# yeyupiaoling/VoiceprintRecognition-PaddlePaddle

Hardware: AMD Instinct MI355X
Metric: utterances/sec (3 s, 16 kHz) ECAPA-TDNN fwd+AAM (higher is better)
Workload: dtype bf16; 1 GPU; BASELINE configs[1]: ECAPA-TDNN (C=512, MFA 1536, ASP, embd 192) + Kaldi Fbank 80, 3 s @ 16 kHz (T=298), 2796-class cosine head + AAMLoss, eval-mode forward, batch 256 per GPU, inputs resident in HBM, random-init weights; batch_per_gpu=256, global_batch=256, parallelism=dp1 (no collective), streams_per_gpu=2, hip_graph=True, graph_prereplays=40

## Files before the change

### include/vpmi.h

```cpp
#ifndef VPMI_H
#define VPMI_H
#include <stddef.h>
#include <stdint.h>

#ifdef __cplusplus
extern "C" {
#endif

#define VPMI_VERSION 100

typedef struct vp_ctx vp_ctx;
typedef void* vp_stream;

enum { VP_OK = 0, VP_EINVAL = -1, VP_ENOMEM = -2, VP_EHIP = -3, VP_EUNSUP = -4, VP_EWORKSPACE = -5 };
enum { VP_F32 = 0, VP_BF16 = 1,
       VP_F32X3 = 2,
       VP_HL32 = 3 };
enum { VP_PAD_NONE = 0, VP_PAD_REFLECT = 1, VP_PAD_ZERO = 2 };
enum { VP_ACT_NONE = 0, VP_ACT_RELU = 1, VP_ACT_SIGMOID = 2, VP_ACT_TANH = 3,
       VP_ACT_HARDTANH20 = 4,
       VP_ACT_SILU = 5 };

int vp_version(void);
vp_ctx* vp_create(int device);
// ... 99 lines not shown
int vp_se_scale_residual(vp_ctx* ctx, int dtype, const void* x, int ldx, int xoff, const float* s,
                         const void* res, int ldr, int roff, void* out, int ldo, int ooff,
                         int B, int T, int C, vp_stream stream);
int vp_se_scale_residual_shadow(vp_ctx* ctx, const float* x, int ldx, int xoff, const float* s, const float* res, int ldr, int roff,
                                float* out, int ldo, int ooff, void* shadow, int ld_shadow, int shadow_off, int B, int T, int C,
                                vp_stream stream);

int vp_asp_softmax_stats(vp_ctx* ctx, int dtype, const float* logits, const void* x, int ldx, int xoff,
                         int B, int T, int C, float eps, float* pooled, vp_stream stream);

#define VP_MAX_SE_BLOCKS 8
#define VP_MAX_RES2 15

typedef struct {
    const void* w;
    const float* bias;
    const float* bn_scale;
    const float* bn_shift;
    int cin, cout, kw, dil;
    const void* w_hl;
} vp_tdnn_layer;

typedef struct {
    vp_tdnn_layer tdnn1;
    vp_tdnn_layer res2[VP_MAX_RES2];
    vp_tdnn_layer tdnn2;
    const float* se_w1;
    const float* se_b1;
    const float* se_w2;
    const float* se_b2;
} vp_se_res2_block;

typedef struct {
    vp_tdnn_layer tdnn;
    const float* w_ctx;
    const void* conv_w;
    const float* conv_b;
    int C, att;
} vp_asp_weights;

typedef struct {
    int dtype;
    int feat_dim, embd_dim, n_blocks, res2_scale, se_ch;
    vp_tdnn_layer block0;
    vp_se_res2_block blk[VP_MAX_SE_BLOCKS];
    vp_tdnn_layer mfa;
    vp_asp_weights asp;
    const float* fc_w;
    const float* fc_b;
} vp_ecapa_weights;

int vp_res2_chain_fwd(vp_ctx* ctx, const vp_tdnn_layer* layers, int nconv, const void* t1, void* r2, int B, int T, int C,
                      int width, vp_stream stream);
int vp_asp_fused_fwd(vp_ctx* ctx, const void* h, const void* w, const float* bias, const void* x, int ldx, const float* center,
                     int ldc, int B, int T, int C, int att, float eps, float* pooled, vp_stream stream);
int vp_se_gate_fwd(vp_ctx* ctx, const float* psum, const float* shift, int B, int T, int C, int H, const float* w1, const float* b1,
                   const float* w2, const float* b2, float* out, vp_stream stream);
int vp_asp_utt_fwd(vp_ctx* ctx, const void* x, int ldx, const vp_tdnn_layer* tdnn, const float* rowbias, const void* conv_w,
                   const float* conv_b, int B, int T, int C, int att, float eps, float* pooled, vp_stream stream);

int vp_res2_chain_x3_fwd(vp_ctx* ctx, const vp_tdnn_layer* layers, int nconv, const void* t1, void* r2, int B, int T, int C,
                         int width, vp_stream stream);
int vp_res2_chain_x3_plan(int T, int nconv, int dil, int* nsplit, int* tseg, int* tp, int* lds_bytes);
int vp_ecapa_x3_fast_path(const vp_ecapa_weights* w, int B, int T);
int vp_asp_fused_x3_fwd(vp_ctx* ctx, const void* h, const float* w, const float* bias, const void* x, int ldx, const float* center,
                        int ldc, int B, int T, int C, int att, float eps, float* pooled, vp_stream stream);

size_t vp_ecapa_workspace_bytes(const vp_ecapa_weights* w, int B, int T);
int vp_ecapa_fwd(vp_ctx* ctx, const vp_ecapa_weights* w, const void* feats, int B, int T, float* emb,
                 void* ws, size_t ws_bytes, vp_stream stream);

typedef struct {
    int dtype;
    int feat_dim, embd_dim, channels;
    vp_tdnn_layer td[5];
    vp_asp_weights asp;
    const float* lin_w;
    const float* lin_b;
} vp_tdnn_weights;

size_t vp_tdnn_workspace_bytes(const vp_tdnn_weights* w, int B, int T);
int vp_tdnn_fwd(vp_ctx* ctx, const vp_tdnn_weights* w, const void* feats, int B, int T, float* emb,
                void* ws, size_t ws_bytes, vp_stream stream);

#define VP_MAX_CAM_LAYERS 64
#define VP_MAX_CAM_BLOCKS 4

typedef struct {
    vp_tdnn_layer conv1, conv2, shortcut;
    int stride, has_shortcut;
} vp_resblock;

typedef struct {
    const float* bn1_scale;
    const float* bn1_shift;
    vp_tdnn_layer linear1;
    vp_tdnn_layer local;
    const float* ctx_w1;
    const float* ctx_b1;
    const float* ctx_w2;
    const float* ctx_b2;
} vp_cam_layer;

typedef struct {
    const float* bn_scale;
    const float* bn_shift;
// ... 422 lines not shown
```

### voiceprintrecognition-paddlepaddle_amd/csrc/common.h

```cpp
#pragma once
#include <hip/hip_runtime.h>
#include <stdint.h>
#include <stdio.h>
#include <string.h>

#include "../../include/vpmi.h"

struct vp_ctx {
    int device;
    char err[512];
    vp_fbank_opts fb_opts;
    int fb_valid;
    int fb_win, fb_shift, fb_nfft, fb_nmel, fb_nnz;
    float* fb_window;
    float2* fb_twiddle;
    int* fb_mel_start;
    int* fb_mel_bin0;
    float* fb_mel_w;
    float* fb_wpad;
    int fb_f16, fb_rounds, fb_wpad_len, fb_round_off[8], fb_round_max[8];
    vp_mel_opts ms_opts;
    int ms_valid, ms_nnz;
    float* ms_window;
    float2* ms_twiddle;
// ... 63 lines not shown
    o[0] = (bf16_t)v[0]; o[1] = (bf16_t)v[1]; o[2] = (bf16_t)v[2]; o[3] = (bf16_t)v[3];
    *reinterpret_cast<bf16x4*>(p) = o;
}

__device__ __forceinline__ float vp_wave_sum(float v) {
#pragma unroll
    for (int o = 32; o > 0; o >>= 1) v += __shfl_xor(v, o);
    return v;
}
__device__ __forceinline__ float vp_wave_max(float v) {
#pragma unroll
    for (int o = 32; o > 0; o >>= 1) v = fmaxf(v, __shfl_xor(v, o));
    return v;
}

__device__ __forceinline__ unsigned vp_order_key(float s) {
    const unsigned u = __float_as_uint(s);
    return u ^ ((u >> 31) ? 0xffffffffu : 0x80000000u);
}

static inline size_t vp_dtype_size(int dt) { return dt == VP_BF16 ? 2 : 4; }
static inline int vp_storage_dtype(int dt) { return dt == VP_F32X3 ? VP_F32 : dt; }
static inline bool vp_backbone_dtype_ok(int dt) { return dt == VP_F32 || dt == VP_BF16 || dt == VP_F32X3; }

#define VP_CONV_BM 128

int vp_dense_f32_ex(vp_ctx* ctx, const float* a, int lda, const float* w, int w_is_kn, const float* bias,
                    const float* rowscale, const float* colscale, int M, int N, int K, int act, float* out,
                    int ldo, hipStream_t st);
int vp_asp_softmax_stats_ex(vp_ctx* ctx, int dtype, const float* logits, const void* x, int ldx, int xoff,
                            const float* center, int ldc, int B, int T, int C, float eps, float* pooled, hipStream_t st);
struct VpAspBufs { void* h; float* e; float* psum; float* psumsq; float* stats; float* rowbias; float* pooled; };
int vp_run_asp(vp_ctx* ctx, const vp_asp_weights& A, int dtype, const void* x, int ldx, const float* shift,
               int B, int T, const VpAspBufs& w, hipStream_t st);
int vp_asp_utt_bf16(vp_ctx* ctx, const void* x, int ldx, const vp_tdnn_layer* tdnn, const float* rowbias, const void* conv_w,
                    const float* conv_b, int B, int T, int C, int att, float eps, float* pooled, hipStream_t st);
void vp_launch_sum_partials(const float* part, int S, long long n, float* out, hipStream_t st, int Cin = 1, int KW = 1, int batch = 1,
                            int KF = 1);
int vp_conv3x3_c1(vp_ctx* ctx, int dtype, const void* feats, void* out, const float* w, const float* bias,
                  const float* scale, const float* shift, int B, int T, int F, int C, hipStream_t st);
int vp_se_scale_residual_ex(vp_ctx* ctx, int dtype, const void* x, int ldx, int xoff, const float* s,
                            const void* res, int ldr, int roff, void* out, int ldo, int ooff, int B, int T, int C,
                            int relu, hipStream_t st);
int vp_im2col_hl32(vp_ctx* ctx, const float* x, int B, int T, int F, int KW, int dil, int pad, void* out, int Kp, hipStream_t st);
int vp_time_moments(vp_ctx* ctx, int dtype, const void* x, int ldx, int B, int T, int C, float eps, int unbiased,
                    float* stats, hipStream_t st);
int vp_se_gate(vp_ctx* ctx, const float* psum, const float* shift, int B, int T, int C, int H, const float* w1, const float* b1,
               const float* w2, const float* b2, float* out, hipStream_t st);
int vp_copy_cols(vp_ctx* ctx, int dtype, const void* x, int ldx, int xoff, void* y, int ldy, int yoff, long long rows, int C,
                 hipStream_t st);
int vp_aff_combine(vp_ctx* ctx, int dtype, const void* t, int ldt, const void* x, int ldx, int xoff, const void* y, int ldy,
                   int yoff, void* o, int ldo, int ooff, long long rows, int C, hipStream_t st);
int vp_res2_chain_bf16(vp_ctx* ctx, const vp_tdnn_layer* layers, int nconv, const void* t1, void* r2, int B, int T,
                       int C, int width, hipStream_t st);
int vp_res2_chain_x3(vp_ctx* ctx, const vp_tdnn_layer* layers, int nconv, const void* t1, void* r2, int B, int T, int C, int width,
                     hipStream_t st);
bool vp_res2_chain_x3_ok(const vp_tdnn_layer* layers, int nconv, int B, int T, int C, int width);
int vp_asp_fused_x3(vp_ctx* ctx, const void* h, const float* w, const float* bias, const void* x, int ldx, const float* center, int ldc,
                    int B, int T, int C, int att, float eps, float* pooled, hipStream_t st);
int vp_asp_fused_bf16(vp_ctx* ctx, const void* h, const void* w, const float* bias, const void* x, int ldx,
                      const float* center, int ldc, int B, int T, int C, int att, float eps, float* pooled,
                      hipStream_t st);
int vp_row_inv_norm(vp_ctx* ctx, const float* x, int rows, int D, int ld, float eps, float* inv, hipStream_t st);
int vp_reduce_rows(vp_ctx* ctx, const float* v, int n, int mean, float* out, hipStream_t st);
int vp_conv3x3_c32_bf16(vp_ctx* ctx, const void* x, void* y, const vp_tdnn_layer* conv, const void* res, int relu,
                        const vp_tdnn_layer* shortcut, void* y2, int B, int T, int F_in, int stride_f, const void* c1_feats,
                        const float* c1_w, const float* c1_b, const float* c1_scale, const float* c1_shift, hipStream_t st);
int vp_resblock_c32_bf16(vp_ctx* ctx, const void* x, void* y, const vp_tdnn_layer* conv1, const vp_tdnn_layer* conv2, int B, int T, int F,
                         hipStream_t st);
int vp_pointwise_bf16(vp_ctx* ctx, const vp_conv1d_desc* d, int only_where_it_wins, hipStream_t st);
int vp_cam_block_bf16(vp_ctx* ctx, const vp_cam_layer* layers, int n_layers, void* cat, int ld, int ch0, int B, int Tn, int seg_len,
                      int bn_channels, int growth, hipStream_t st);

int vp_fbank_release_tables(vp_ctx* ctx);
int vp_mel_release_tables(vp_ctx* ctx);
int vp_reverb_release_tables(vp_ctx* ctx);

template <typename TO>
__device__ __forceinline__ float vp_tanh_for(float x) {
    if constexpr (sizeof(TO) == 2) {
        const float e = __builtin_amdgcn_exp2f(x * 2.8853900817779268f);
        return 1.f - 2.f * __builtin_amdgcn_rcpf(e + 1.f);
    } else {
        return tanhf(x);
    }
}

template <typename TO>
__device__ __forceinline__ float vp_silu_for(float x) {
    if constexpr (sizeof(TO) == 2) return x * __builtin_amdgcn_rcpf(1.f + __builtin_amdgcn_exp2f(x * -1.4426950408889634f));
    else return x / (1.f + __expf(-x));
}
```

### voiceprintrecognition-paddlepaddle_amd/csrc/ecapa.hip

```cpp
#include "launch.h"

#include <stdlib.h>

namespace {

void tdnn_desc(vp_conv1d_desc& d, const vp_tdnn_layer& L, int dtype, int B, int T_in, int T_out, int pad_mode) {
    vp_layer_desc(d, L, dtype, pad_mode);
    vp_geom_rows(d, B, T_in, T_out);
    d.dilation = L.dil; d.pad_left = pad_mode == VP_PAD_NONE ? 0 : L.dil * (L.kw - 1) / 2;
    d.act = VP_ACT_RELU; d.ldx = d.ldy = 0;
}

}

int vp_run_asp(vp_ctx* ctx, const vp_asp_weights& A, int dtc, const void* x, int ldx, const float* shift,
               int B, int T, const VpAspBufs& w, hipStream_t st) {
    const int C = A.C;
    const int dtype = vp_storage_dtype(dtc);
    int rc = VP_OK;
    if (w.psum) rc = vp_moments_finalize(ctx, w.psum, w.psumsq, shift, B, T, C, 1e-12f, 1, w.stats, st);
    if (rc) return rc;
    if (A.w_ctx) {
        rc = vp_dense_f32_ex(ctx, w.stats, 2 * C, A.w_ctx, 0, nullptr, nullptr, nullptr, B, A.att, 2 * C, VP_ACT_NONE,
                             w.rowbias, A.att, st);
// ... 112 lines not shown
    auto hl_layer = [&](const vp_tdnn_layer& L) {
        tdnn_desc(d, L, VP_F32X3, B, T, T, VP_PAD_REFLECT);
        d.dtype_in = d.dtype_out = VP_HL32; d.w = L.w_hl; d.mfma_bf16 = 2;
    };
    const int Kp0 = (int)vp_align_up((size_t)w->block0.kw * w->block0.cin, 32);
    if (w->block0.w_hl && p.im && w->feat_dim == w->block0.cin && w->block0.cin % 8 == 0) {
        const int pad = w->block0.dil * (w->block0.kw - 1) / 2;
        if ((rc = vp_im2col_hl32(ctx, (const float*)feats, B, T, w->block0.cin, w->block0.kw, w->block0.dil, pad, p.im, Kp0, st))) return rc;
        tdnn_desc(d, w->block0, VP_F32X3, B, T, T, VP_PAD_REFLECT);
        d.dtype_in = d.dtype_out = VP_HL32; d.w = w->block0.w_hl; d.mfma_bf16 = 2;
        d.Cin = Kp0; d.KW = 1; d.dilation = 1; d.pad_left = 0;
        d.x = p.im; d.ldx = Kp0; d.y = p.cat0; d.ldy = C;
    } else {
        tdnn_desc(d, w->block0, VP_F32X3, B, T, T, VP_PAD_REFLECT);
        d.dtype_out = VP_HL32; d.w = w->block0.w; d.mfma_bf16 = 2;
        d.x = feats; d.ldx = w->feat_dim; d.y = p.cat0; d.ldy = C;
    }
    if ((rc = vp_conv1d_fwd(ctx, &d, st))) return rc;
    const void* xin = p.cat0;
    int ld_in = C, off_in = 0;
    for (int i = 0; i < nb; ++i) {
        const vp_se_res2_block& blk = w->blk[i];
        hl_layer(blk.tdnn1);
        d.x = xin; d.ldx = ld_in; d.xoff = off_in; d.y = p.t1; d.ldy = C;
        d.y2 = p.r2; d.ldy2 = C; d.y2off = 0; d.ysplit = width;
        if ((rc = vp_conv1d_fwd(ctx, &d, st))) return rc;
        rc = vp_res2_chain_x3(ctx, blk.res2, sc - 1, p.t1, p.r2, B, T, C, width, st);
        if (rc == VP_EUNSUP) VP_FAIL(ctx, VP_EUNSUP, "ecapa: Res2 chain left the split-precision kernel's range after the shape check");
        if (rc) return rc;
        hl_layer(blk.tdnn2);
        d.x = p.r2; d.ldx = C; d.xoff = 0; d.y = p.t2; d.ldy = C; d.psum = p.psum;
        if ((rc = vp_conv1d_fwd(ctx, &d, st))) return rc;
        if ((rc = vp_se_gate(ctx, p.psum, blk.tdnn2.bn_shift, B, T, C, w->se_ch, blk.se_w1, blk.se_b1, blk.se_w2, blk.se_b2, p.se_s, st)))
            return rc;
        if ((rc = vp_se_scale_residual_ex(ctx, VP_HL32, p.t2, C, 0, p.se_s, xin, ld_in, off_in, p.cat, ldcat, i * C, B, T, C, 0, st))) return rc;
        xin = p.cat; ld_in = ldcat; off_in = i * C;
    }
    hl_layer(w->mfa);
    d.x = p.cat; d.ldx = ldcat; d.y = p.mfa; d.ldy = Cm; d.psum = p.psum; d.psumsq = p.psumsq;
    if ((rc = vp_conv1d_fwd(ctx, &d, st))) return rc;
    VpAspBufs ab{p.h, p.e, p.psum, p.psumsq, p.stats, p.rowbias, p.pooled};
    if ((rc = vp_run_asp(ctx, w->asp, VP_HL32, p.mfa, Cm, w->mfa.bn_shift, B, T, ab, st))) return rc;
    return vp_dense_f32_ex(ctx, p.pooled, 2 * Cm, w->fc_w, 0, w->fc_b, nullptr, nullptr, B, w->embd_dim, 2 * Cm,
                           VP_ACT_NONE, emb, w->embd_dim, st);
}

}

extern "C" {

int vp_res2_chain_fwd(vp_ctx* ctx, const vp_tdnn_layer* layers, int nconv, const void* t1, void* r2, int B, int T, int C,
                      int width, vp_stream stream) {
    if (!ctx || !layers || !t1 || !r2 || B <= 0 || T <= 0 || C <= 0) VP_FAIL(ctx, VP_EINVAL, "res2_chain: bad arguments");
    const int rc = vp_res2_chain_bf16(ctx, layers, nconv, t1, r2, B, T, C, width, (hipStream_t)stream);
    if (rc == VP_EUNSUP) VP_FAIL(ctx, VP_EUNSUP, "res2_chain: shape not covered by the fused kernel (width 64, equal dilations, 2 <= T <= 384)");
    return rc;
}

int vp_asp_utt_fwd(vp_ctx* ctx, const void* x, int ldx, const vp_tdnn_layer* tdnn, const float* rowbias, const void* conv_w,
                   const float* conv_b, int B, int T, int C, int att, float eps, float* pooled, vp_stream stream) {
    if (!ctx || !x || !tdnn || !conv_w || !pooled || B <= 0) VP_FAIL(ctx, VP_EINVAL, "asp_utt: bad arguments");
    const int rc = vp_asp_utt_bf16(ctx, x, ldx, tdnn, rowbias, conv_w, conv_b, B, T, C, att, eps, pooled, (hipStream_t)stream);
    if (rc == VP_EUNSUP) VP_FAIL(ctx, VP_EUNSUP, "asp_utt: shape not covered (attention width 128, C %% 64 == 0, T <= 304, 1x1 TDNN with BatchNorm)");
    return rc;
}

int vp_asp_fused_fwd(vp_ctx* ctx, const void* h, const void* w, const float* bias, const void* x, int ldx, const float* center,
                     int ldc, int B, int T, int C, int att, float eps, float* pooled, vp_stream stream) {
    if (!ctx || !h || !w || !x || !center || !pooled || B <= 0) VP_FAIL(ctx, VP_EINVAL, "asp_fused: bad arguments");
    const int rc = vp_asp_fused_bf16(ctx, h, w, bias, x, ldx, center, ldc, B, T, C, att, eps, pooled, (hipStream_t)stream);
    if (rc == VP_EUNSUP) VP_FAIL(ctx, VP_EUNSUP, "asp_fused: shape not covered (attention width 128, C and ldx multiples of 8, 16-byte aligned)");
    return rc;
}

int vp_res2_chain_x3_fwd(vp_ctx* ctx, const vp_tdnn_layer* layers, int nconv, const void* t1, void* r2, int B, int T, int C,
                         int width, vp_stream stream) {
    if (!ctx || !layers || !t1 || !r2 || B <= 0 || T <= 0 || C <= 0) VP_FAIL(ctx, VP_EINVAL, "res2_chain_x3: bad arguments");
    const int rc = vp_res2_chain_x3(ctx, layers, nconv, t1, r2, B, T, C, width, (hipStream_t)stream);
    if (rc == VP_EUNSUP) VP_FAIL(ctx, VP_EUNSUP, "res2_chain_x3: shape not covered (width 64, equal dilations, split weights present, segments fit the LDS)");
    return rc;
}

int vp_asp_fused_x3_fwd(vp_ctx* ctx, const void* h, const float* w, const float* bias, const void* x, int ldx, const float* center,
                        int ldc, int B, int T, int C, int att, float eps, float* pooled, vp_stream stream) {
    if (!ctx || !h || !w || !bias || !x || !pooled || B <= 0) VP_FAIL(ctx, VP_EINVAL, "asp_fused_x3: bad arguments");
    const int rc = vp_asp_fused_x3(ctx, h, w, bias, x, ldx, center, ldc, B, T, C, att, eps, pooled, (hipStream_t)stream);
    if (rc == VP_EUNSUP) VP_FAIL(ctx, VP_EUNSUP, "asp_fused_x3: shape not covered (attention width 128, C and ldx multiples of 32, 16-byte aligned)");
    return rc;
}

int vp_se_gate_fwd(vp_ctx* ctx, const float* psum, const float* shift, int B, int T, int C, int H, const float* w1, const float* b1,
                   const float* w2, const float* b2, float* out, vp_stream stream) {
    return vp_se_gate(ctx, psum, shift, B, T, C, H, w1, b1, w2, b2, out, (hipStream_t)stream);
}

int vp_ecapa_x3_fast_path(const vp_ecapa_weights* w, int B, int T) {
    if (!w || B <= 0 || T <= 0 || w->dtype != VP_F32X3 || w->n_blocks < 1 || w->n_blocks > VP_MAX_SE_BLOCKS || w->res2_scale < 2 ||
        w->res2_scale - 1 > VP_MAX_RES2)
        return 0;
    return ecapa_hl_ok(w, B, T) ? 1 : 0;
}

size_t vp_ecapa_workspace_bytes(const vp_ecapa_weights* w, int B, int T) {
    if (!w || B <= 0 || T <= 0) return 0;
    EcapaPlan p;
    plan_ecapa(w, B, T, nullptr, p);
    return p.total;
}

int vp_ecapa_fwd(vp_ctx* ctx, const vp_ecapa_weights* w, const void* feats, int B, int T, float* emb,
                 void* ws, size_t ws_bytes, vp_stream stream) {
    if (!ctx || !w || !feats || !emb || B <= 0 || T <= 0) VP_FAIL(ctx, VP_EINVAL, "ecapa: bad arguments");
    int rc = check_ecapa(ctx, w);
    if (rc) return rc;
    EcapaPlan p;
    plan_ecapa(w, B, T, ws, p);
    if (!ws || ws_bytes < p.total) VP_FAIL(ctx, VP_EWORKSPACE, "ecapa: workspace %zu < %zu", ws_bytes, p.total);
    hipStream_t st = (hipStream_t)stream;
    const int dtc = w->dtype, dt = vp_storage_dtype(dtc);
    const int C = w->block0.cout, Cm = w->mfa.cout, nb = w->n_blocks, sc = w->res2_scale;
    const int width = C / sc, ldcat = nb * C;
    vp_conv1d_desc d;
    if (dtc == VP_F32X3 && ecapa_hl_ok(w, B, T)) return ecapa_fwd_hl(ctx, w, feats, B, T, emb, p, st);

    tdnn_desc(d, w->block0, dtc, B, T, T, VP_PAD_REFLECT);
    d.x = feats; d.ldx = w->feat_dim; d.y = p.cat0; d.ldy = C;
    if ((rc = vp_conv1d_fwd(ctx, &d, st))) return rc;

    const void* xin = p.cat0;
    int ld_in = C, off_in = 0;
    for (int i = 0; i < nb; ++i) {
        const vp_se_res2_block& blk = w->blk[i];
        tdnn_desc(d, blk.tdnn1, dtc, B, T, T, VP_PAD_REFLECT);
        d.x = xin; d.ldx = ld_in; d.xoff = off_in; d.y = p.t1; d.ldy = C;
        d.y2 = p.r2; d.ldy2 = C; d.y2off = 0; d.ysplit = width;
        if ((rc = vp_conv1d_fwd(ctx, &d, st))) return rc;
        int fused = VP_EUNSUP;
        static const bool res2_unfused = getenv("VPMI_RES2_UNFUSED") != nullptr;
        if (dt == VP_BF16 && !res2_unfused) fused = vp_res2_chain_bf16(ctx, blk.res2, sc - 1, p.t1, p.r2, B, T, C, width, st);
        if (fused != VP_OK && fused != VP_EUNSUP) return fused;
        void* tin = nullptr;
        void* tout = p.tmpA;
        for (int j = 1; j < sc && fused != VP_OK; ++j) {
            tdnn_desc(d, blk.res2[j - 1], dtc, B, T, T, VP_PAD_REFLECT);
            if (j == 1) { d.x = p.t1; d.ldx = C; d.xoff = width; }
            else { d.x = tin; d.ldx = width; d.xoff = 0; }
            d.y = p.r2; d.ldy = C; d.yoff = j * width;
            if (j + 1 < sc) {
                d.add_in = p.t1; d.ld_add = C; d.add_off = (j + 1) * width;
                d.aux = tout; d.ld_aux = width; d.aux_off = 0;
            }
            if ((rc = vp_conv1d_fwd(ctx, &d, st))) return rc;
            tin = tout;
            tout = (tout == p.tmpA) ? p.tmpB : p.tmpA;
        }
        tdnn_desc(d, blk.tdnn2, dtc, B, T, T, VP_PAD_REFLECT);
        d.x = p.r2; d.ldx = C; d.xoff = 0;
        d.y = p.t2; d.ldy = C; d.psum = p.psum;
        if ((rc = vp_conv1d_fwd(ctx, &d, st))) return rc;
        if ((rc = vp_se_gate(ctx, p.psum, blk.tdnn2.bn_shift, B, T, C, w->se_ch, blk.se_w1, blk.se_b1, blk.se_w2, blk.se_b2,
                             p.se_s, st))) return rc;
        if ((rc = vp_se_scale_residual(ctx, dt, p.t2, C, 0, p.se_s, xin, ld_in, off_in, p.cat, ldcat, i * C, B, T, C, st)))
            return rc;
        xin = p.cat; ld_in = ldcat; off_in = i * C;
    }
    tdnn_desc(d, w->mfa, dtc, B, T, T, VP_PAD_REFLECT);
    d.x = p.cat; d.ldx = ldcat; d.y = p.mfa; d.ldy = Cm; d.psum = p.psum; d.psumsq = p.psumsq;
    if ((rc = vp_conv1d_fwd(ctx, &d, st))) return rc;
    VpAspBufs ab{p.h, p.e, p.psum, p.psumsq, p.stats, p.rowbias, p.pooled};
    if ((rc = vp_run_asp(ctx, w->asp, dtc, p.mfa, Cm, w->mfa.bn_shift, B, T, ab, st))) return rc;
    return vp_dense_f32_ex(ctx, p.pooled, 2 * Cm, w->fc_w, 0, w->fc_b, nullptr, nullptr, B, w->embd_dim, 2 * Cm,
                           VP_ACT_NONE, emb, w->embd_dim, st);
}

static void tdnn_T(const vp_tdnn_weights* w, int T, int Ts[6]) {
    Ts[0] = T;
    for (int i = 0; i < 5; ++i) Ts[i + 1] = Ts[i] - w->td[i].dil * (w->td[i].kw - 1);
}

struct TdnnPlan { void* a; void* b; void* h; float *e, *psum, *psumsq, *stats, *rowbias, *pooled; size_t total; };

static void plan_tdnn(const vp_tdnn_weights* w, int B, int T, void* ws, TdnnPlan& p) {
    const size_t es = vp_dtype_size(w->dtype);
    const int C = w->channels;
    int Ts[6];
    tdnn_T(w, T, Ts);
    const int T1 = Ts[1] > 0 ? Ts[1] : 1, T5 = Ts[5] > 0 ? Ts[5] : 1;
    Carver c(ws);
    p.a = c.take((size_t)B * T1 * C * es);
    p.b = c.take((size_t)B * T1 * C * es);
    p.h = c.take((size_t)B * T5 * w->asp.att * es);
    p.e = (float*)c.take((size_t)B * T5 * C * sizeof(float));
// ... 48 lines not shown
```

### voiceprintrecognition-paddlepaddle_amd/csrc/res2_chain.hip

```cpp
#include "common.h"

namespace {

constexpr int R2_W = 64;
constexpr int R2_K = 3 * R2_W;
constexpr int R2_THREADS = 512;
constexpr int R2_WAVES = R2_THREADS / 64;
constexpr int R2_ROUNDS = 3;
typedef __attribute__((address_space(3))) void* r2_lds_ptr;

struct Res2Args {
    const bf16_t* t1;
    bf16_t* r2;
    const bf16_t* w[VP_MAX_RES2];
    const float* bias[VP_MAX_RES2];
    const float* scale[VP_MAX_RES2];
    const float* shift[VP_MAX_RES2];
    int T, C, nconv, dil, TP;
    unsigned t1_bytes;
#ifdef VP_TIMING
    unsigned long long* dbg;
#endif
};

__device__ __forceinline__ int reflect_idx(int t, int T) {
    t = t < 0 ? -t : t;
    return t >= T ? 2 * (T - 1) - t : t;
}

__global__ __launch_bounds__(R2_THREADS, 1) void res2_chain_kernel(Res2Args a) {
    extern __shared__ __attribute__((aligned(16))) char smem[];
    const int act_bytes = a.TP * 128;
    char* act0 = smem;
    char* wt0 = smem + 2 * act_bytes;
    constexpr int WT_BYTES = R2_W * R2_K * 2;
#ifdef VP_TIMING
    unsigned long long stamps[32];
    int nst = 0;
    stamps[nst++] = wall_clock64();
#endif
    const int tid = threadIdx.x, lane = tid & 63;
    const int wv = __builtin_amdgcn_readfirstlane(tid >> 6);
    const int li = lane & 15, g = lane >> 4;
    const int b = blockIdx.x;
    const size_t row0 = (size_t)b * a.T;
    constexpr unsigned OOB = 0xfffffff0u;
    const __amdgpu_buffer_rsrc_t xsrd = __builtin_amdgcn_make_buffer_rsrc(const_cast<bf16_t*>(a.t1), 0, a.t1_bytes, 0x00020000);

    const int drow = lane >> 3;
    const unsigned dchunk = (unsigned)((lane & 7) ^ drow) << 4;
    auto dma_x = [&](int slice, char* dst) {
        const unsigned colb = (unsigned)slice * (R2_W * 2) + dchunk;
        for (int p = wv; p < a.TP / 8; p += R2_WAVES) {
            const int t = p * 8 + drow;
            const unsigned off = t < a.T ? (unsigned)((row0 + t) * a.C * 2) + colb : OOB;
            __builtin_amdgcn_raw_ptr_buffer_load_lds(xsrd, (r2_lds_ptr)(dst + p * 1024), 16, off, 0, 0, 0);
        }
    };
    auto dma_w = [&](int j, char* dst) {
        const __amdgpu_buffer_rsrc_t wsrd = __builtin_amdgcn_make_buffer_rsrc(const_cast<bf16_t*>(a.w[j]), 0, WT_BYTES, 0x00020000);
#pragma unroll
        for (int u = 0; u < 3; ++u) {
            const int p = wv + u * R2_WAVES;
            const int tap = p >> 3, nb = (p & 7) * 8;
            const unsigned off = (unsigned)((nb + drow) * (R2_K * 2) + tap * 128) + dchunk;
            __builtin_amdgcn_raw_ptr_buffer_load_lds(wsrd, (r2_lds_ptr)(dst + tap * 8192 + nb * 128), 16, off, 0, 0, 0);
        }
    };

    dma_x(1, act0);
    dma_w(0, wt0);
    const int ntile = a.TP / 16;
    float* prm = reinterpret_cast<float*>(wt0 + 2 * WT_BYTES);
    for (int i = tid; i < a.nconv * 192; i += R2_THREADS) {
        const int j = i / 192, k = i - j * 192, which = k >> 6, n = k & 63;
        prm[i] = which == 0 ? a.bias[j][n] : (which == 1 ? a.scale[j][n] : a.shift[j][n]);
    }
    asm volatile("s_waitcnt vmcnt(0)" ::: "memory");
    __syncthreads();
#ifdef VP_TIMING
    stamps[nst++] = wall_clock64();
#endif

    for (int j = 0; j < a.nconv; ++j) {
        char* ain = act0 + (j & 1) * act_bytes;
        char* aout = act0 + ((j + 1) & 1) * act_bytes;
        const char* wl = wt0 + (j & 1) * WT_BYTES;
        const bool has_next = j + 1 < a.nconv;
        if (has_next) {
            dma_x(j + 2, aout);
            dma_w(j + 1, wt0 + ((j + 1) & 1) * WT_BYTES);
        }
        bf16x8 wf[4][6];
#pragma unroll
        for (int ni = 0; ni < 4; ++ni) {
            const int n = ni * 16 + li;
#pragma unroll
            for (int s = 0; s < 6; ++s) {
                const int c = (s & 1) * 4 + g;
                wf[ni][s] = *reinterpret_cast<const bf16x8*>(wl + (s >> 1) * 8192 + n * 128 + ((c ^ (n & 7)) << 4));
            }
        }
        f32x4 acc[R2_ROUNDS][4];
#pragma unroll
        for (int r = 0; r < R2_ROUNDS; ++r) {
            const int mt = wv + r * R2_WAVES;
            const int t = min(mt * 16 + li, a.TP - 1);
#pragma unroll
            for (int ni = 0; ni < 4; ++ni) acc[r][ni] = f32x4{0.f, 0.f, 0.f, 0.f};
#pragma unroll
            for (int tap = 0; tap < 3; ++tap) {
                int ts = reflect_idx(t + (tap - 1) * a.dil, a.T);
                ts = min(max(ts, 0), a.TP - 1);
#pragma unroll
                for (int ks = 0; ks < 2; ++ks) {
                    const int c = ks * 4 + g;
                    const bf16x8 xf = *reinterpret_cast<const bf16x8*>(ain + ts * 128 + ((c ^ (ts & 7)) << 4));
#pragma unroll
                    for (int ni = 0; ni < 4; ++ni)
                        acc[r][ni] = __builtin_amdgcn_mfma_f32_16x16x32_bf16(wf[ni][tap * 2 + ks], xf, acc[r][ni], 0, 0, 0);
                }
            }
        }
#ifdef VP_TIMING
        if (nst < 32) stamps[nst++] = wall_clock64();
#endif
        asm volatile("s_waitcnt vmcnt(0)" ::: "memory");
        __syncthreads();
#ifdef VP_TIMING
        if (nst < 32) stamps[nst++] = wall_clock64();
#endif
        const float* pj = prm + j * 192;
#pragma unroll
        for (int r = 0; r < R2_ROUNDS; ++r) {
            const int mt = wv + r * R2_WAVES;
            if (mt < ntile) {
                const int t = mt * 16 + li;
#pragma unroll
                for (int ni = 0; ni < 4; ++ni) {
                    const int nb = ni * 16 + g * 4;
                    const float4 bb = *reinterpret_cast<const float4*>(pj + nb);
                    const float4 ss = *reinterpret_cast<const float4*>(pj + 64 + nb);
                    const float4 hh = *reinterpret_cast<const float4*>(pj + 128 + nb);
                    float v[4];
                    v[0] = fmaxf(acc[r][ni][0] + bb.x, 0.f) * ss.x + hh.x;
                    v[1] = fmaxf(acc[r][ni][1] + bb.y, 0.f) * ss.y + hh.y;
                    v[2] = fmaxf(acc[r][ni][2] + bb.z, 0.f) * ss.z + hh.z;
                    v[3] = fmaxf(acc[r][ni][3] + bb.w, 0.f) * ss.w + hh.w;
                    const int pos = t * 128 + (((nb >> 3) ^ (t & 7)) << 4) + (nb & 7) * 2;
                    bf16x4 o;
                    o[0] = (bf16_t)v[0]; o[1] = (bf16_t)v[1]; o[2] = (bf16_t)v[2]; o[3] = (bf16_t)v[3];
                    *reinterpret_cast<bf16x4*>(ain + pos) = o;
                    if (has_next) {
                        const bf16x4 xn = *reinterpret_cast<const bf16x4*>(aout + pos);
                        bf16x4 s;
                        s[0] = (bf16_t)(v[0] + (float)xn[0]); s[1] = (bf16_t)(v[1] + (float)xn[1]);
                        s[2] = (bf16_t)(v[2] + (float)xn[2]); s[3] = (bf16_t)(v[3] + (float)xn[3]);
                        *reinterpret_cast<bf16x4*>(aout + pos) = s;
                    }
                }
            }
        }
        __syncthreads();
#ifdef VP_TIMING
        if (nst < 32) stamps[nst++] = wall_clock64();
#endif
        {
            bf16_t* ybase = a.r2 + row0 * a.C + (j + 1) * R2_W;
            for (int i = tid; i < a.T * 8; i += R2_THREADS) {
                const int t = i >> 3, c = i & 7;
                const uint4 v = *reinterpret_cast<const uint4*>(ain + t * 128 + ((c ^ (t & 7)) << 4));
                *reinterpret_cast<uint4*>(ybase + (size_t)t * a.C + c * 8) = v;
            }
        }
        __syncthreads();
#ifdef VP_TIMING
        if (nst < 32) stamps[nst++] = wall_clock64();
#endif
    }
#ifdef VP_TIMING
    if (a.dbg && tid == 0)
        for (int i = 0; i < 32; ++i) a.dbg[(size_t)b * 32 + i] = i < nst ? stamps[i] : 0;
#endif
}

}

#ifdef VP_TIMING
static unsigned long long* g_res2_dbg = nullptr;
extern "C" void vp_dbg_res2_buffer(void* p) { g_res2_dbg = (unsigned long long*)p; }
#endif

int vp_res2_chain_bf16(vp_ctx* ctx, const vp_tdnn_layer* layers, int nconv, const void* t1, void* r2, int B, int T,
                       int C, int width, hipStream_t st) {
    if (width != R2_W || nconv < 1 || nconv > VP_MAX_RES2) return VP_EUNSUP;
    const int TP = (T + 15) / 16 * 16;
    const size_t smem = (size_t)2 * TP * 128 + 2 * (size_t)R2_W * R2_K * 2 + (size_t)nconv * 192 * 4;
    if (smem > 160 * 1024 || T < 2 || TP / 16 > R2_WAVES * R2_ROUNDS) return VP_EUNSUP;
    const int dil = layers[0].dil;
    Res2Args a;
    memset(&a, 0, sizeof(a));
    for (int j = 0; j < nconv; ++j) {
        const vp_tdnn_layer& L = layers[j];
        if (L.kw != 3 || L.cin != R2_W || L.cout != R2_W || L.dil != dil || !L.bias || !L.bn_scale || !L.bn_shift)
            return VP_EUNSUP;
        a.w[j] = (const bf16_t*)L.w; a.bias[j] = L.bias; a.scale[j] = L.bn_scale; a.shift[j] = L.bn_shift;
    }
    if (dil >= T) return VP_EUNSUP;
    a.t1 = (const bf16_t*)t1; a.r2 = (bf16_t*)r2; a.T = T; a.C = C; a.nconv = nconv; a.dil = dil; a.TP = TP;
    const unsigned long long t1b = (unsigned long long)B * T * C * 2;
    if (t1b >= 0xffffff00ull || (C * 2) % 16 || (reinterpret_cast<uintptr_t>(t1) | reinterpret_cast<uintptr_t>(r2)) & 15) return VP_EUNSUP;
    a.t1_bytes = (unsigned)t1b;
#ifdef VP_TIMING
    a.dbg = g_res2_dbg;
#endif
    static bool attr_dev[64] = {};
    bool& attr_set = attr_dev[ctx->device & 63];
    if (!attr_set) {
        VP_HIP(ctx, hipFuncSetAttribute(reinterpret_cast<const void*>(res2_chain_kernel),
                                        hipFuncAttributeMaxDynamicSharedMemorySize, 160 * 1024));
        attr_set = true;
    }
    hipLaunchKernelGGL(res2_chain_kernel, dim3(B), dim3(R2_THREADS), smem, st, a);
    VP_LAUNCH_CHECK(ctx, "res2_chain");
    return VP_OK;
}
```

Baseline: 206,100 utterances/s.

## Split res2 chain kernel into halo-padded time segments to fit two blocks per CU

```diff
diff --git a/include/vpmi.h b/include/vpmi.h
--- a/include/vpmi.h
+++ b/include/vpmi.h
@@ -175,6 +175,9 @@
 
 int vp_res2_chain_fwd(vp_ctx* ctx, const vp_tdnn_layer* layers, int nconv, const void* t1, void* r2, int B, int T, int C,
                       int width, vp_stream stream);
+int vp_res2_chain_seg_fwd(vp_ctx* ctx, const vp_tdnn_layer* layers, int nconv, const void* t1, void* r2, int B, int T, int C,
+                          int width, int nsplit, vp_stream stream);
+int vp_res2_chain_plan(int T, int nconv, int dil, int* nsplit, int* tseg, int* tp, int* lds_bytes);
 int vp_asp_fused_fwd(vp_ctx* ctx, const void* h, const void* w, const float* bias, const void* x, int ldx, const float* center,
                      int ldc, int B, int T, int C, int att, float eps, float* pooled, vp_stream stream);
 int vp_se_gate_fwd(vp_ctx* ctx, const float* psum, const float* shift, int B, int T, int C, int H, const float* w1, const float* b1,
diff --git a/voiceprintrecognition-paddlepaddle_amd/csrc/common.h b/voiceprintrecognition-paddlepaddle_amd/csrc/common.h
--- a/voiceprintrecognition-paddlepaddle_amd/csrc/common.h
+++ b/voiceprintrecognition-paddlepaddle_amd/csrc/common.h
@@ -139,7 +139,7 @@
 int vp_aff_combine(vp_ctx* ctx, int dtype, const void* t, int ldt, const void* x, int ldx, int xoff, const void* y, int ldy,
                    int yoff, void* o, int ldo, int ooff, long long rows, int C, hipStream_t st);
 int vp_res2_chain_bf16(vp_ctx* ctx, const vp_tdnn_layer* layers, int nconv, const void* t1, void* r2, int B, int T,
-                       int C, int width, hipStream_t st);
+                       int C, int width, int nsplit, hipStream_t st);
 int vp_res2_chain_x3(vp_ctx* ctx, const vp_tdnn_layer* layers, int nconv, const void* t1, void* r2, int B, int T, int C, int width,
                      hipStream_t st);
 bool vp_res2_chain_x3_ok(const vp_tdnn_layer* layers, int nconv, int B, int T, int C, int width);
diff --git a/voiceprintrecognition-paddlepaddle_amd/csrc/ecapa.hip b/voiceprintrecognition-paddlepaddle_amd/csrc/ecapa.hip
--- a/voiceprintrecognition-paddlepaddle_amd/csrc/ecapa.hip
+++ b/voiceprintrecognition-paddlepaddle_amd/csrc/ecapa.hip
@@ -188,8 +188,17 @@
 int vp_res2_chain_fwd(vp_ctx* ctx, const vp_tdnn_layer* layers, int nconv, const void* t1, void* r2, int B, int T, int C,
                       int width, vp_stream stream) {
     if (!ctx || !layers || !t1 || !r2 || B <= 0 || T <= 0 || C <= 0) VP_FAIL(ctx, VP_EINVAL, "res2_chain: bad arguments");
-    const int rc = vp_res2_chain_bf16(ctx, layers, nconv, t1, r2, B, T, C, width, (hipStream_t)stream);
+    const int rc = vp_res2_chain_bf16(ctx, layers, nconv, t1, r2, B, T, C, width, 0, (hipStream_t)stream);
     if (rc == VP_EUNSUP) VP_FAIL(ctx, VP_EUNSUP, "res2_chain: shape not covered by the fused kernel (width 64, equal dilations, 2 <= T <= 384)");
+    return rc;
+}
+
+int vp_res2_chain_seg_fwd(vp_ctx* ctx, const vp_tdnn_layer* layers, int nconv, const void* t1, void* r2, int B, int T, int C,
+                          int width, int nsplit, vp_stream stream) {
+    if (!ctx || !layers || !t1 || !r2 || B <= 0 || T <= 0 || C <= 0 || nsplit < 0) VP_FAIL(ctx, VP_EINVAL, "res2_chain_seg: bad arguments");
+    const int rc = vp_res2_chain_bf16(ctx, layers, nconv, t1, r2, B, T, C, width, nsplit, (hipStream_t)stream);
+    if (rc == VP_EUNSUP)
+        VP_FAIL(ctx, VP_EUNSUP, "res2_chain_seg: shape or segment count not covered (width 64, equal dilations, 2 <= T <= 384, held window <= 192 frames)");
     return rc;
 }
 
@@ -273,7 +282,7 @@
         if ((rc = vp_conv1d_fwd(ctx, &d, st))) return rc;
         int fused = VP_EUNSUP;
         static const bool res2_unfused = getenv("VPMI_RES2_UNFUSED") != nullptr;
-        if (dt == VP_BF16 && !res2_unfused) fused = vp_res2_chain_bf16(ctx, blk.res2, sc - 1, p.t1, p.r2, B, T, C, width, st);
+        if (dt == VP_BF16 && !res2_unfused) fused = vp_res2_chain_bf16(ctx, blk.res2, sc - 1, p.t1, p.r2, B, T, C, width, 0, st);
         if (fused != VP_OK && fused != VP_EUNSUP) return fused;
         void* tin = nullptr;
         void* tout = p.tmpA;
diff --git a/voiceprintrecognition-paddlepaddle_amd/csrc/res2_chain.hip b/voiceprintrecognition-paddlepaddle_amd/csrc/res2_chain.hip
--- a/voiceprintrecognition-paddlepaddle_amd/csrc/res2_chain.hip
+++ b/voiceprintrecognition-paddlepaddle_amd/csrc/res2_chain.hip
@@ -4,10 +4,17 @@
 
 constexpr int R2_W = 64;
 constexpr int R2_K = 3 * R2_W;
-constexpr int R2_THREADS = 512;
+constexpr int R2_THREADS = 384;
 constexpr int R2_WAVES = R2_THREADS / 64;
-constexpr int R2_ROUNDS = 3;
+constexpr int R2_ROUNDS = 2;
+constexpr int R2_TP_MAX = 16 * R2_WAVES * R2_ROUNDS;
+constexpr int R2_WT_BYTES = R2_W * R2_K * 2;
+constexpr int R2_PRM_BYTES = 3 * R2_W * 4;
+constexpr int R2_LDS_MAX = 80 * 1024;
+constexpr int R2_T_MAX = 384;
 typedef __attribute__((address_space(3))) void* r2_lds_ptr;
+
+struct R2Plan { int nsplit, Tseg, TP, H, lds; };
 
 struct Res2Args {
     const bf16_t* t1;
@@ -16,7 +23,7 @@
     const float* bias[VP_MAX_RES2];
     const float* scale[VP_MAX_RES2];
     const float* shift[VP_MAX_RES2];
-    int T, C, nconv, dil, TP;
+    int T, C, nconv, dil, TP, Tseg, H, nsplit;
     unsigned t1_bytes;
 #ifdef VP_TIMING
     unsigned long long* dbg;
@@ -28,12 +35,14 @@
     return t >= T ? 2 * (T - 1) - t : t;
 }
 
-__global__ __launch_bounds__(R2_THREADS, 1) void res2_chain_kernel(Res2Args a) {
+__global__ __launch_bounds__(R2_THREADS, 4) void res2_chain_kernel(Res2Args a) {
     extern __shared__ __attribute__((aligned(16))) char smem[];
-    const int act_bytes = a.TP * 128;
+    __builtin_amdgcn_s_setprio(3);
+    const int TP = a.TP;
+    const int act_bytes = TP * 128;
     char* act0 = smem;
-    char* wt0 = smem + 2 * act_bytes;
-    constexpr int WT_BYTES = R2_W * R2_K * 2;
+    char* wts = smem + 2 * act_bytes;
+    float* prm = reinterpret_cast<float*>(wts + R2_WT_BYTES);
 #ifdef VP_TIMING
     unsigned long long stamps[32];
     int nst = 0;
@@ -42,36 +51,38 @@
     const int tid = threadIdx.x, lane = tid & 63;
     const int wv = __builtin_amdgcn_readfirstlane(tid >> 6);
     const int li = lane & 15, g = lane >> 4;
-    const int b = blockIdx.x;
+    const int b = blockIdx.x / a.nsplit, seg = blockIdx.x - b * a.nsplit;
+    const int own0 = seg * a.Tseg, own1 = min(a.T, own0 + a.Tseg);
+    const int lo = max(0, own0 - a.H), hi = min(a.T, own1 + a.H);
+    const int rows = hi - lo;
     const size_t row0 = (size_t)b * a.T;
     constexpr unsigned OOB = 0xfffffff0u;
     const __amdgpu_buffer_rsrc_t xsrd = __builtin_amdgcn_make_buffer_rsrc(const_cast<bf16_t*>(a.t1), 0, a.t1_bytes, 0x00020000);
 
     const int drow = lane >> 3;
     const unsigned dchunk = (unsigned)((lane & 7) ^ drow) << 4;
+    const unsigned wvoff = (unsigned)(drow * (R2_K * 2)) + dchunk;
     auto dma_x = [&](int slice, char* dst) {
         const unsigned colb = (unsigned)slice * (R2_W * 2) + dchunk;
-        for (int p = wv; p < a.TP / 8; p += R2_WAVES) {
-            const int t = p * 8 + drow;
-            const unsigned off = t < a.T ? (unsigned)((row0 + t) * a.C * 2) + colb : OOB;
+        for (int p = wv; p < TP / 8; p += R2_WAVES) {
+            const int r = p * 8 + drow;
+            const unsigned off = r < rows ? (unsigned)((row0 + lo + r) * a.C * 2) + colb : OOB;
             __builtin_amdgcn_raw_ptr_buffer_load_lds(xsrd, (r2_lds_ptr)(dst + p * 1024), 16, off, 0, 0, 0);
         }
     };
-    auto dma_w = [&](int j, char* dst) {
-        const __amdgpu_buffer_rsrc_t wsrd = __builtin_amdgcn_make_buffer_rsrc(const_cast<bf16_t*>(a.w[j]), 0, WT_BYTES, 0x00020000);
-#pragma unroll
-        for (int u = 0; u < 3; ++u) {
-            const int p = wv + u * R2_WAVES;
-            const int tap = p >> 3, nb = (p & 7) * 8;
-            const unsigned off = (unsigned)((nb + drow) * (R2_K * 2) + tap * 128) + dchunk;
-            __builtin_amdgcn_raw_ptr_buffer_load_lds(wsrd, (r2_lds_ptr)(dst + tap * 8192 + nb * 128), 16, off, 0, 0, 0);
+    auto dma_w = [&](int j, int tap) {
+        const __amdgpu_buffer_rsrc_t wsrd = __builtin_amdgcn_make_buffer_rsrc(const_cast<bf16_t*>(a.w[j]), 0, R2_WT_BYTES, 0x00020000);
+#pragma unroll
+        for (int p = wv; p < R2_W / 8; p += R2_WAVES) {
+            const int nb = p * 8;
+            __builtin_amdgcn_raw_ptr_buffer_load_lds(wsrd, (r2_lds_ptr)(wts + tap * 8192 + nb * 128), 16, wvoff,
+                                                     nb * (R2_K * 2) + tap * 128, 0, 0);
         }
     };
 
     dma_x(1, act0);
-    dma_w(0, wt0);
-    const int ntile = a.TP / 16;
-    float* prm = reinterpret_cast<float*>(wt0 + 2 * WT_BYTES);
+    dma_w(0, 0); dma_w(0, 1); dma_w(0, 2);
+    const int ntile = TP / 16;
     for (int i = tid; i < a.nconv * 192; i += R2_THREADS) {
         const int j = i / 192, k = i - j * 192, which = k >> 6, n = k & 63;
         prm[i] = which == 0 ? a.bias[j][n] : (which == 1 ? a.scale[j][n] : a.shift[j][n]);
@@ -82,43 +93,73 @@
     stamps[nst++] = wall_clock64();
 #endif
 
+    bool on[R2_ROUNDS];
+    int trow[R2_ROUNDS];
+#pragma unroll
+    for (int r = 0; r < R2_ROUNDS; ++r) {
+        const int mt = wv + r * R2_WAVES;
+        on[r] = mt < ntile;
+        trow[r] = mt * 16 + li;
+    }
+    const int r0 = own0 - lo, r1 = own1 - lo;
+    const int ct = wv * 16 + (lane >> 3);
+    const int clds = ct * 128 + (((lane & 7) ^ (ct & 7)) << 4);
+    const unsigned ldy = (unsigned)a.C * 2u, cglb = (unsigned)ct * ldy + (unsigned)(lane & 7) * 16u;
+
     for (int j = 0; j < a.nconv; ++j) {
         char* ain = act0 + (j & 1) * act_bytes;
         char* aout = act0 + ((j + 1) & 1) * act_bytes;
-        const char* wl = wt0 + (j & 1) * WT_BYTES;
         const bool has_next = j + 1 < a.nconv;
-        if (has_next) {
-            dma_x(j + 2, aout);
-            dma_w(j + 1, wt0 + ((j + 1) & 1) * WT_BYTES);
-        }
-        bf16x8 wf[4][6];
-#pragma unroll
-        for (int ni = 0; ni < 4; ++ni) {
-            const int n = ni * 16 + li;
-#pragma unroll
-            for (int s = 0; s < 6; ++s) {
-                const int c = (s & 1) * 4 + g;
-                wf[ni][s] = *reinterpret_cast<const bf16x8*>(wl + (s >> 1) * 8192 + n * 128 + ((c ^ (n & 7)) << 4));
-            }
+        if (has_next) dma_x(j + 2, aout);
+        int trd[R2_ROUNDS][3];
+#pragma unroll
+        for (int r = 0; r < R2_ROUNDS; ++r) {
+            const int tl = min(trow[r], rows - 1);
+#pragma unroll
+            for (int tap = 0; tap < 3; ++tap)
+                trd[r][tap] = min(max(reflect_idx(lo + tl + (tap - 1) * a.dil, a.T) - lo, 0), rows - 1);
         }
         f32x4 acc[R2_ROUNDS][4];
 #pragma unroll
-        for (int r = 0; r < R2_ROUNDS; ++r) {
-            const int mt = wv + r * R2_WAVES;
-            const int t = min(mt * 16 + li, a.TP - 1);
+        for (int r = 0; r < R2_ROUNDS; ++r)
 #pragma unroll
             for (int ni = 0; ni < 4; ++ni) acc[r][ni] = f32x4{0.f, 0.f, 0.f, 0.f};
 #pragma unroll
-            for (int tap = 0; tap < 3; ++tap) {
-                int ts = reflect_idx(t + (tap - 1) * a.dil, a.T);
-                ts = min(max(ts, 0), a.TP - 1);
+        for (int tap = 0; tap < 3; ++tap) {
+            bf16x8 wf[4][2];
+#pragma unroll
+            for (int ni = 0; ni < 4; ++ni) {
+                const int n = ni * 16 + li;
 #pragma unroll
                 for (int ks = 0; ks < 2; ++ks) {
                     const int c = ks * 4 + g;
-                    const bf16x8 xf = *reinterpret_cast<const bf16x8*>(ain + ts * 128 + ((c ^ (ts & 7)) << 4));
-#pragma unroll
-                    for (int ni = 0; ni < 4; ++ni)
-                        acc[r][ni] = __builtin_amdgcn_mfma_f32_16x16x32_bf16(wf[ni][tap * 2 + ks], xf, acc[r][ni], 0, 0, 0);
+                    wf[ni][ks] = *reinterpret_cast<const bf16x8*>(wts + tap * 8192 + n * 128 + ((c ^ (n & 7)) << 4));
+                }
+            }
+            bf16x8 xf[R2_ROUNDS][2];
+#pragma unroll
+            for (int r = 0; r < R2_ROUNDS; ++r) {
+                const int ts = on[r] ? trd[r][tap] : 0;
+#pragma unroll
+                for (int ks = 0; ks < 2; ++ks) {
+                    const int c = ks * 4 + g;
+                    xf[r][ks] = *reinterpret_cast<const bf16x8*>(ain + ts * 128 + ((c ^ (ts & 7)) << 4));
+                }
+            }
+            if (has_next) {
+                asm volatile("s_waitcnt lgkmcnt(0)" ::: "memory");
+                __builtin_amdgcn_s_barrier();
+                asm volatile("" ::: "memory");
+                dma_w(j + 1, tap);
+            }
+#pragma unroll
+            for (int r = 0; r < R2_ROUNDS; ++r) {
+                if (on[r]) {
+#pragma unroll
+                    for (int ks = 0; ks < 2; ++ks)
+#pragma unroll
+                        for (int ni = 0; ni < 4; ++ni)
+                            acc[r][ni] = __builtin_amdgcn_mfma_f32_16x16x32_bf16(wf[ni][ks], xf[r][ks], acc[r][ni], 0, 0, 0);
                 }
             }
         }
@@ -132,56 +173,104 @@
 #endif
         const float* pj = prm + j * 192;
 #pragma unroll
-        for (int r = 0; r < R2_ROUNDS; ++r) {
-            const int mt = wv + r * R2_WAVES;
-            if (mt < ntile) {
-                const int t = mt * 16 + li;
-#pragma unroll
-                for (int ni = 0; ni < 4; ++ni) {
-                    const int nb = ni * 16 + g * 4;
-                    const float4 bb = *reinterpret_cast<const float4*>(pj + nb);
-                    const float4 ss = *reinterpret_cast<const float4*>(pj + 64 + nb);
-                    const float4 hh = *reinterpret_cast<const float4*>(pj + 128 + nb);
-                    float v[4];
-                    v[0] = fmaxf(acc[r][ni][0] + bb.x, 0.f) * ss.x + hh.x;
-                    v[1] = fmaxf(acc[r][ni][1] + bb.y, 0.f) * ss.y + hh.y;
-                    v[2] = fmaxf(acc[r][ni][2] + bb.z, 0.f) * ss.z + hh.z;
-                    v[3] = fmaxf(acc[r][ni][3] + bb.w, 0.f) * ss.w + hh.w;
-                    const int pos = t * 128 + (((nb >> 3) ^ (t & 7)) << 4) + (nb & 7) * 2;
-                    bf16x4 o;
-                    o[0] = (bf16_t)v[0]; o[1] = (bf16_t)v[1]; o[2] = (bf16_t)v[2]; o[3] = (bf16_t)v[3];
-                    *reinterpret_cast<bf16x4*>(ain + pos) = o;
-                    if (has_next) {
-                        const bf16x4 xn = *reinterpret_cast<const bf16x4*>(aout + pos);
-                        bf16x4 s;
-                        s[0] = (bf16_t)(v[0] + (float)xn[0]); s[1] = (bf16_t)(v[1] + (float)xn[1]);
-                        s[2] = (bf16_t)(v[2] + (float)xn[2]); s[3] = (bf16_t)(v[3] + (float)xn[3]);
-                        *reinterpret_cast<bf16x4*>(aout + pos) = s;
+        for (int half = 0; half < 2; ++half) {
+            float4 bb[2], ss[2], hh[2];
+            int pos[R2_ROUNDS][2];
+            bf16x4 xn[R2_ROUNDS][2];
+#pragma unroll
+            for (int q = 0; q < 2; ++q) {
+                const int nb = (half * 2 + q) * 16 + g * 4;
+                bb[q] = *reinterpret_cast<const float4*>(pj + nb);
+                ss[q] = *reinterpret_cast<const float4*>(pj + 64 + nb);
+                hh[q] = *reinterpret_cast<const float4*>(pj + 128 + nb);
+#pragma unroll
+                for (int r = 0; r < R2_ROUNDS; ++r) {
+                    const int t = trow[r];
+                    pos[r][q] = t * 128 + (((nb >> 3) ^ (t & 7)) << 4) + (nb & 7) * 2;
+                    xn[r][q] = bf16x4{0, 0, 0, 0};
+                    if (on[r] && has_next) xn[r][q] = *reinterpret_cast<const bf16x4*>(aout + pos[r][q]);
+                }
+            }
+#pragma unroll
+            for (int r = 0; r < R2_ROUNDS; ++r) {
+                if (on[r]) {
+#pragma unroll
+                    for (int q = 0; q < 2; ++q) {
+                        const f32x4 ac = acc[r][half * 2 + q];
+                        float v[4];
+                        v[0] = fmaxf(ac[0] + bb[q].x, 0.f) * ss[q].x + hh[q].x;
+                        v[1] = fmaxf(ac[1] + bb[q].y, 0.f) * ss[q].y + hh[q].y;
+                        v[2] = fmaxf(ac[2] + bb[q].z, 0.f) * ss[q].z + hh[q].z;
+                        v[3] = fmaxf(ac[3] + bb[q].w, 0.f) * ss[q].w + hh[q].w;
+                        bf16x4 o;
+                        o[0] = (bf16_t)v[0]; o[1] = (bf16_t)v[1]; o[2] = (bf16_t)v[2]; o[3] = (bf16_t)v[3];
+                        *reinterpret_cast<bf16x4*>(ain + pos[r][q]) = o;
+                        if (has_next) {
+                            bf16x4 s;
+                            s[0] = (bf16_t)(v[0] + (float)xn[r][q][0]); s[1] = (bf16_t)(v[1] + (float)xn[r][q][1]);
+                            s[2] = (bf16_t)(v[2] + (float)xn[r][q][2]); s[3] = (bf16_t)(v[3] + (float)xn[r][q][3]);
+                            *reinterpret_cast<bf16x4*>(aout + pos[r][q]) = s;
+                        }
                     }
                 }
             }
         }
-        __syncthreads();
+        {
+            char* ybase = reinterpret_cast<char*>(a.r2 + (row0 + lo) * a.C + (j + 1) * R2_W);
+#pragma unroll
+            for (int r = 0; r < R2_ROUNDS; ++r) {
+                if (on[r]) {
+#pragma unroll
+                    for (int h = 0; h < 2; ++h) {
+                        const int dt = r * R2_WAVES * 16 + h * 8;
+                        if (ct + dt >= r0 && ct + dt < r1) {
+                            const uint4 v = *reinterpret_cast<const uint4*>(ain + clds + dt * 128);
+                            *reinterpret_cast<uint4*>(ybase + (cglb + (unsigned)dt * ldy)) = v;
+                        }
+                    }
+                }
+            }
+        }
 #ifdef VP_TIMING
         if (nst < 32) stamps[nst++] = wall_clock64();
 #endif
-        {
-            bf16_t* ybase = a.r2 + row0 * a.C + (j + 1) * R2_W;
-            for (int i = tid; i < a.T * 8; i += R2_THREADS) {
-                const int t = i >> 3, c = i & 7;
-                const uint4 v = *reinterpret_cast<const uint4*>(ain + t * 128 + ((c ^ (t & 7)) << 4));
-                *reinterpret_cast<uint4*>(ybase + (size_t)t * a.C + c * 8) = v;
-            }
-        }
-        __syncthreads();
+        asm volatile("s_waitcnt lgkmcnt(0)" ::: "memory");
+        __builtin_amdgcn_s_barrier();
+        asm volatile("" ::: "memory");
 #ifdef VP_TIMING
         if (nst < 32) stamps[nst++] = wall_clock64();
 #endif
     }
 #ifdef VP_TIMING
     if (a.dbg && tid == 0)
-        for (int i = 0; i < 32; ++i) a.dbg[(size_t)b * 32 + i] = i < nst ? stamps[i] : 0;
-#endif
+        for (int i = 0; i < 32; ++i) a.dbg[(size_t)blockIdx.x * 32 + i] = i < nst ? stamps[i] : 0;
+#endif
+}
+
+bool r2_plan_for(int T, int nconv, int dil, int ns, R2Plan& p) {
+    p = R2Plan{};
+    if (T < 2 || T > R2_T_MAX || nconv < 1 || nconv > VP_MAX_RES2 || dil < 1 || dil >= T || ns < 1 || ns > T) return false;
+    const int H = nconv * dil;
+    const int ts = (T + ns - 1) / ns;
+    if ((ns - 1) * ts >= T) return false;
+    int need = 0;
+    for (int s = 0; s < ns; ++s) {
+        const int o0 = s * ts, o1 = T < o0 + ts ? T : o0 + ts;
+        const int l = o0 - H > 0 ? o0 - H : 0, h = o1 + H < T ? o1 + H : T;
+        need = h - l > need ? h - l : need;
+    }
+    const int tp = (need + 15) / 16 * 16;
+    const int lds = 2 * tp * 128 + R2_WT_BYTES + nconv * R2_PRM_BYTES;
+    if (tp > R2_TP_MAX || lds > R2_LDS_MAX) return false;
+    p.nsplit = ns; p.Tseg = ts; p.TP = tp; p.H = H; p.lds = lds;
+    return true;
+}
+
+bool r2_plan(int T, int nconv, int dil, R2Plan& p) {
+    for (int ns = 1; ns <= T && ns <= R2_T_MAX; ++ns)
+        if (r2_plan_for(T, nconv, dil, ns, p)) return true;
+    p = R2Plan{};
+    return false;
 }
 
 }
@@ -192,12 +281,13 @@
 #endif
 
 int vp_res2_chain_bf16(vp_ctx* ctx, const vp_tdnn_layer* layers, int nconv, const void* t1, void* r2, int B, int T,
-                       int C, int width, hipStream_t st) {
-    if (width != R2_W || nconv < 1 || nconv > VP_MAX_RES2) return VP_EUNSUP;
-    const int TP = (T + 15) / 16 * 16;
-    const size_t smem = (size_t)2 * TP * 128 + 2 * (size_t)R2_W * R2_K * 2 + (size_t)nconv * 192 * 4;
-    if (smem > 160 * 1024 || T < 2 || TP / 16 > R2_WAVES * R2_ROUNDS) return VP_EUNSUP;
+                       int C, int width, int nsplit, hipStream_t st) {
+    if (width != R2_W || nconv < 1 || nconv > VP_MAX_RES2 || T < 2 || T > R2_T_MAX || B < 1 || nsplit < 0 ||
+        C < (nconv + 1) * R2_W)
+        return VP_EUNSUP;
     const int dil = layers[0].dil;
+    R2Plan p;
+    if (!(nsplit ? r2_plan_for(T, nconv, dil, nsplit, p) : r2_plan(T, nconv, dil, p))) return VP_EUNSUP;
     Res2Args a;
     memset(&a, 0, sizeof(a));
     for (int j = 0; j < nconv; ++j) {
@@ -206,22 +296,36 @@
             return VP_EUNSUP;
         a.w[j] = (const bf16_t*)L.w; a.bias[j] = L.bias; a.scale[j] = L.bn_scale; a.shift[j] = L.bn_shift;
     }
-    if (dil >= T) return VP_EUNSUP;
-    a.t1 = (const bf16_t*)t1; a.r2 = (bf16_t*)r2; a.T = T; a.C = C; a.nconv = nconv; a.dil = dil; a.TP = TP;
+    a.t1 = (const bf16_t*)t1; a.r2 = (bf16_t*)r2; a.T = T; a.C = C; a.nconv = nconv; a.dil = dil;
+    a.TP = p.TP; a.Tseg = p.Tseg; a.H = p.H; a.nsplit = p.nsplit;
     const unsigned long long t1b = (unsigned long long)B * T * C * 2;
     if (t1b >= 0xffffff00ull || (C * 2) % 16 || (reinterpret_cast<uintptr_t>(t1) | reinterpret_cast<uintptr_t>(r2)) & 15) return VP_EUNSUP;
     a.t1_bytes = (unsigned)t1b;
 #ifdef VP_TIMING
     a.dbg = g_res2_dbg;
 #endif
-    static bool attr_dev[64] = {};
-    bool& attr_set = attr_dev[ctx->device & 63];
-    if (!attr_set) {
+    static signed char two_fit[64] = {};
+    signed char& fit = two_fit[ctx->device & 63];
+    if (!fit) {
         VP_HIP(ctx, hipFuncSetAttribute(reinterpret_cast<const void*>(res2_chain_kernel),
-                                        hipFuncAttributeMaxDynamicSharedMemorySize, 160 * 1024));
-        attr_set = true;
-    }
-    hipLaunchKernelGGL(res2_chain_kernel, dim3(B), dim3(R2_THREADS), smem, st, a);
+                                        hipFuncAttributeMaxDynamicSharedMemorySize, R2_LDS_MAX));
+        int nb = 0;
+        VP_HIP(ctx, hipOccupancyMaxActiveBlocksPerMultiprocessor(&nb, reinterpret_cast<const void*>(res2_chain_kernel), R2_THREADS,
+                                                                 R2_LDS_MAX));
+        fit = nb >= 2 ? 1 : -1;
+    }
+    if (fit < 0) return VP_EUNSUP;
+    hipLaunchKernelGGL(res2_chain_kernel, dim3((unsigned)B * p.nsplit), dim3(R2_THREADS), p.lds, st, a);
     VP_LAUNCH_CHECK(ctx, "res2_chain");
     return VP_OK;
 }
+
+extern "C" int vp_res2_chain_plan(int T, int nconv, int dil, int* nsplit, int* tseg, int* tp, int* lds_bytes) {
+    R2Plan p;
+    const bool ok = r2_plan(T, nconv, dil, p);
+    if (nsplit) *nsplit = p.nsplit;
+    if (tseg) *tseg = p.Tseg;
+    if (tp) *tp = p.TP;
+    if (lds_bytes) *lds_bytes = p.lds;
+    return ok ? VP_OK : VP_EUNSUP;
+}
```

Result: no change. 204,400 utterances/s (-0.8%).
